# tky823/DNN-based_source_separation

Hardware: NVIDIA H100
Metric: audio-sec/s Conv-TasNet 2spk 4s@8kHz fwd+SI-SDR-PIT (higher is better)
Workload: dtype f32 via 3xFP16 split on wgmma (f16), fp32 accumulate

## Files before the change

### dnn-based_source_separation_b200/csrc/ctn_wgmma.cu

```cuda
#include "ctn_internal.h"
#include "ctn_wgmma_ptx.cuh"
#include "ctn_dw_math.cuh"
#include <cuda_fp16.h>
#include <stdlib.h>
#include <string.h>

int ctn_pw_simt(const PwArgs& a, int pro, int epi, cudaStream_t st);

namespace {

constexpr int TM = 128;
constexpr int KS = 32;
constexpr int NT = 128;
constexpr int THREADS = 256;
constexpr int CPW = 4;
constexpr int STAGES = 2;
constexpr int SMEM_HEADER = 1024;
constexpr int F16_MAX_ROWS = 2048;

template <int PRO, int EPI, bool F16>
__host__ __device__ constexpr bool chan_split() { return F16 && (PRO == PRO_DW || EPI == EPI_H); }
template <int PRO, int EPI, bool F16>
__host__ __device__ constexpr int tile_frames() { return chan_split<PRO, EPI, F16>() ? 64 : TM; }

struct TcArgs {
  PwArgs a;
  const float* wimg;
  const float* oscale;
  int n_tiles, k_slabs, t_tiles;
  int n_groups;
  int nt_per_cta;
};

template <int PRO>
__host__ __device__ constexpr int raw_q() { return PRO == PRO_DW ? 3 : PRO == PRO_RES ? 2 : 1; }
template <int PRO, int CPT>
struct Raw { float4 q[CPT][raw_q<PRO>()]; };

template <int PRO, int CPT>
__device__ __forceinline__ void load_raw(const PwArgs& a, int b, int c0, int tbase, int first, int step, bool interior, Raw<PRO, CPT>& r) {
#pragma unroll
  for (int j = 0; j < CPT; ++j) {
    const int c = c0 + j;
    if constexpr (PRO == PRO_DW) {
      const int cc = interior ? c : (c < a.K ? c : a.K - 1);
      const float* hr = a.A + ((size_t)b * a.K + cc) * a.pitch;
#pragma unroll
      for (int k = 0; k < 3; ++k) {
        int ts = first + k * step;
        if (!interior) ts = ts < 0 ? 0 : (ts > a.pitch - 4 ? a.pitch - 4 : ts);
        r.q[j][k] = __ldg(reinterpret_cast<const float4*>(hr + ts));
      }
    } else {
      const bool ok = c < a.K;
      r.q[j][0] = ok ? __ldg(reinterpret_cast<const float4*>(a.A + ((size_t)b * a.K + c) * a.pitch + tbase)) : make_float4(0.f, 0.f, 0.f, 0.f);
      if constexpr (PRO == PRO_RES)
        r.q[j][1] = ok ? __ldg(reinterpret_cast<const float4*>(a.res_r + ((size_t)b * a.res_Mt + c) * a.pitch + tbase))
                       : make_float4(0.f, 0.f, 0.f, 0.f);
    }
  }
}

template <int DCLS, bool INTERIOR, bool TRAIN, int CPT>
__device__ __forceinline__ void dw_form(const PwArgs& a, int b, int c0, int tbase, int first, int step, float2 mr1, float pslope,
                                        bool store_side, Raw<PRO_DW, CPT>& r, float4 (&v)[CPT], float2& dls, float2& dlss) {
  const float islope = TRAIN ? __ldg(a.dw_in_slope) : 0.f;
#pragma unroll
  for (int j = 0; j < CPT; ++j) {
    const int c = c0 + j;
    const int cc = INTERIOR ? c : (c < a.K ? c : a.K - 1);
    float4* q = r.q[j];
    if (TRAIN) {
#pragma unroll
      for (int k = 0; k < 3; ++k) {
        q[k].x = prelu_f(q[k].x, islope); q[k].y = prelu_f(q[k].y, islope); q[k].z = prelu_f(q[k].z, islope); q[k].w = prelu_f(q[k].w, islope);
      }
    }
    const float pg = __ldg(a.dw_norm_g + cc), pb = __ldg(a.dw_norm_b + cc), pbd = __ldg(a.dw_b + cc);
    const float w0 = __ldg(a.dw_w + cc * 3), w1 = __ldg(a.dw_w + cc * 3 + 1), w2 = __ldg(a.dw_w + cc * 3 + 2);
    const float gsc = pg * mr1.y, gsh = pb - mr1.x * mr1.y * pg;
    float4 pre;
    v[j] = dw_channel<DCLS, INTERIOR, TRAIN>(q[0], q[1], q[2], gsc, gsh, w0, w1, w2, pbd, pslope, first, step, tbase, a.frames, c < a.K,
                                             dls, dlss, &pre);
    if (TRAIN && store_side && c < a.K) *reinterpret_cast<float4*>(a.dw_u_pre_out + ((size_t)b * a.K + c) * a.pitch + tbase) = pre;
  }
}

template <int PRO, int EPI, int NPASS, bool F16, bool TRAIN>
__global__ void __launch_bounds__(THREADS, F16 ? 2 : 1) k_pw_wgmma(const TcArgs g) {
  constexpr bool CSPLIT = chan_split<PRO, EPI, F16>();
  constexpr int TMC = tile_frames<PRO, EPI, F16>();
  constexpr int NWG = CSPLIT ? 2 : 1;
  constexpr int LPR = TMC / 4;
  constexpr int CPT = CPW * LPR / 32;
  constexpr int NPREC = NPASS == 3 ? 2 : 1;
  constexpr uint32_t ROWB = F16 ? 64u : 128u;
  constexpr uint32_t A_BYTES = TMC * ROWB, W_BYTES = NT * ROWB;
  constexpr uint32_t STAGE_BYTES = NPREC * (A_BYTES + NWG * W_BYTES);
  static_assert(F16 || CPT == CPW, "the K-major tf32 store takes a warp's 4 channels per time step");
  extern __shared__ uint8_t smem_raw[];
  const uint32_t raw = ptx::smem_u32(smem_raw);
  const uint32_t base = (raw + 1023u) & ~1023u;
  uint8_t* smem = smem_raw + (base - raw);
  uint64_t* wbar = reinterpret_cast<uint64_t*>(smem);
  const uint32_t stage0 = base + SMEM_HEADER;
  const int warp = threadIdx.x >> 5, lane = threadIdx.x & 31, wg = warp >> 2;
  const PwArgs& a = g.a;

  const int n_groups = g.n_groups;
  const int ngrp = (int)blockIdx.x % n_groups;
  const int tt = ((int)blockIdx.x / n_groups) % g.t_tiles;
  const int b = (int)blockIdx.x / (n_groups * g.t_tiles);

  if (threadIdx.x == 0) {
    for (int s = 0; s < STAGES; ++s) ptx::mbar_init(ptx::smem_u32(&wbar[s]), 1);
    ptx::fence_mbar_init();
  }
  __syncthreads();

  float act_s = 1.f;
  if (F16 && a.act_scale) act_s = __ldg(a.act_scale);
  float pslope = 0.f;
  if (PRO == PRO_PRELU || PRO == PRO_DW) pslope = __ldg(a.pro_slope);
  const int c_thr = warp * CPW + (lane / LPR) * CPT;
  const int tbase = tt * TMC + (lane % LPR) * 4;
  float2 mr1 = make_float2(0.f, 1.f), mr_res = make_float2(0.f, 1.f);
  if (PRO == PRO_DW) mr1 = gln_mean_rstd(a.dw_stats_in + 2 * b, (double)a.K * (double)a.frames, a.dw_eps);
  if (PRO == PRO_RES) mr_res = gln_mean_rstd(a.res_stats + 2 * b, a.res_n, a.res_eps);
  int dcls = 4, first = tbase, step = 0;
  bool dw_interior = false;
  if (PRO == PRO_DW) {
    const int d = a.dw_dilation;
    dcls = d >= 4 ? 4 : d;
    step = dcls == 4 ? d : 4;
    first = dcls == 4 ? tbase - a.dw_pad_left : tbase - 4;
    const int reach = d >= 4 ? d : 4;
    dw_interior = (tt * TMC - reach >= 0) && (tt * TMC + TMC - 1 + reach + 3 < a.frames) && (a.K % KS == 0) && (a.dw_pad_left == d);
  }

  for (int ntl = 0; ntl < g.nt_per_cta; ++ntl) {
  const int nt0 = CSPLIT ? 2 * ngrp : ngrp * g.nt_per_cta + ntl;
  const int nt = CSPLIT ? nt0 + wg : nt0;
  const bool wg_live = nt < g.n_tiles;
  const int nw = CSPLIT ? min(2, g.n_tiles - nt0) : 1;
  const bool store_side = nt0 == 0;
  const uint8_t* wsrc = reinterpret_cast<const uint8_t*>(g.wimg) + (size_t)nt0 * g.k_slabs * NPREC * W_BYTES;
  float2 dls = make_float2(0.f, 0.f), dlss = make_float2(0.f, 0.f);
  float acc[64];
#pragma unroll
  for (int i = 0; i < 64; ++i) acc[i] = 0.f;

  Raw<PRO, CPT> cur;
  load_raw<PRO, CPT>(a, b, c_thr, tbase, first, step, dw_interior, cur);
  for (int ks = 0; ks < g.k_slabs; ++ks) {
    const int gk = ntl * g.k_slabs + ks;
    const int s = gk & 1;
    const uint32_t st_base = stage0 + (uint32_t)s * STAGE_BYTES;
    if (threadIdx.x == 0) {
      const uint32_t fb = ptx::smem_u32(&wbar[s]);
      ptx::mbar_arrive_expect_tx(fb, (uint32_t)nw * NPREC * W_BYTES);
      for (int w = 0; w < nw; ++w)
        ptx::bulk_g2s(st_base + NPREC * (A_BYTES + w * W_BYTES), wsrc + ((size_t)w * g.k_slabs + ks) * NPREC * W_BYTES, NPREC * W_BYTES, fb);
    }
    const int c0 = ks * KS + c_thr;
    float4 v[CPT];
    if constexpr (PRO == PRO_DW) {
      if (dw_interior) {
        if (dcls == 4) dw_form<4, true, TRAIN>(a, b, c0, tbase, first, step, mr1, pslope, store_side, cur, v, dls, dlss);
        else if (dcls == 2) dw_form<2, true, TRAIN>(a, b, c0, tbase, first, step, mr1, pslope, store_side, cur, v, dls, dlss);
        else dw_form<1, true, TRAIN>(a, b, c0, tbase, first, step, mr1, pslope, store_side, cur, v, dls, dlss);
      } else {
        if (dcls == 4) dw_form<4, false, TRAIN>(a, b, c0, tbase, first, step, mr1, pslope, store_side, cur, v, dls, dlss);
        else if (dcls == 2) dw_form<2, false, TRAIN>(a, b, c0, tbase, first, step, mr1, pslope, store_side, cur, v, dls, dlss);
        else dw_form<1, false, TRAIN>(a, b, c0, tbase, first, step, mr1, pslope, store_side, cur, v, dls, dlss);
      }
    } else {
#pragma unroll
      for (int j = 0; j < CPT; ++j) v[j] = cur.q[j][0];
      if (PRO == PRO_RES) {
#pragma unroll
        for (int j = 0; j < CPT; ++j) {
          const int k = c0 + j;
          const int kc = k < a.K ? k : a.K - 1;
          const float4 r = cur.q[j][PRO == PRO_RES ? 1 : 0];
          const float cst = __ldg(a.res_v1 + kc) - mr_res.x * mr_res.y * __ldg(a.res_v2 + kc);
          float4 xn;
          xn.x = fmaf(mr_res.y, r.x, v[j].x + cst); xn.y = fmaf(mr_res.y, r.y, v[j].y + cst);
          xn.z = fmaf(mr_res.y, r.z, v[j].z + cst); xn.w = fmaf(mr_res.y, r.w, v[j].w + cst);
          if (tbase + 0 >= a.frames) xn.x = 0.f;
          if (tbase + 1 >= a.frames) xn.y = 0.f;
          if (tbase + 2 >= a.frames) xn.z = 0.f;
          if (tbase + 3 >= a.frames) xn.w = 0.f;
          if (k >= a.K) xn = make_float4(0.f, 0.f, 0.f, 0.f);
          v[j] = xn;
          if (store_side && k < a.K) *reinterpret_cast<float4*>(a.res_x_out + ((size_t)b * a.K + k) * a.pitch + tbase) = xn;
        }
      }
      if (PRO == PRO_PRELU) {
#pragma unroll
        for (int j = 0; j < CPT; ++j) {
          v[j].x = prelu_f(v[j].x, pslope); v[j].y = prelu_f(v[j].y, pslope);
          v[j].z = prelu_f(v[j].z, pslope); v[j].w = prelu_f(v[j].w, pslope);
        }
      }
    }
    if (ks + 1 < g.k_slabs) load_raw<PRO, CPT>(a, b, (ks + 1) * KS + c_thr, tbase, first, step, dw_interior, cur);
    uint8_t* sa = smem + SMEM_HEADER + (size_t)s * STAGE_BYTES;
    if (F16) {
      const uint32_t f = (uint32_t)(tbase - tt * TMC);
#pragma unroll
      for (int j = 0; j < CPT; ++j) {
        const uint32_t c = (uint32_t)(c_thr + j);
        const uint32_t off = (f >> 6) * 4096u + (c >> 3) * 1024u + (c & 7) * 128u + ((((f >> 3) & 7) ^ (c & 7)) << 4) + (f & 7) * 2u;
        uint2 h2, l2;
        ptx::split_f16x2(v[j].x * act_s, v[j].y * act_s, h2.x, l2.x);
        ptx::split_f16x2(v[j].z * act_s, v[j].w * act_s, h2.y, l2.y);
        *reinterpret_cast<uint2*>(sa + off) = h2;
        *reinterpret_cast<uint2*>(sa + A_BYTES + off) = l2;
      }
    } else {
#pragma unroll
      for (int e = 0; e < 4; ++e) {
        const int t = lane * 4 + e;
        float x[CPW];
#pragma unroll
        for (int j = 0; j < CPW; ++j) x[j] = e == 0 ? v[j].x : e == 1 ? v[j].y : e == 2 ? v[j].z : v[j].w;
        const uint32_t off = (uint32_t)t * 128u + (((uint32_t)warp ^ (uint32_t)(t & 7)) << 4);
        float4 hi, lo;
        hi.x = ptx::hi_tf32(x[0]); hi.y = ptx::hi_tf32(x[1]); hi.z = ptx::hi_tf32(x[2]); hi.w = ptx::hi_tf32(x[3]);
        lo.x = x[0] - hi.x; lo.y = x[1] - hi.y; lo.z = x[2] - hi.z; lo.w = x[3] - hi.w;
        *reinterpret_cast<float4*>(sa + off) = hi;
        if (NPASS == 3) *reinterpret_cast<float4*>(sa + A_BYTES + off) = lo;
      }
    }
    ptx::fence_proxy_async_smem();
    __syncthreads();
    ptx::mbar_wait(ptx::smem_u32(&wbar[s]), (uint32_t)(gk >> 1) & 1u);
    if (wg_live) {
      const uint32_t a_hi = st_base + (CSPLIT ? 0u : (uint32_t)wg * 64u * ROWB), a_lo = a_hi + A_BYTES;
      const uint32_t w_hi = st_base + NPREC * (A_BYTES + (CSPLIT ? (uint32_t)wg * W_BYTES : 0u)), w_lo = w_hi + W_BYTES;
      ptx::wg_fence();
#pragma unroll
      for (int kk = 0; kk < (F16 ? KS / 16 : KS / 8); ++kk) {
        if (F16) {
          const uint64_t dah = ptx::wg_desc_mn128(a_hi + kk * 2048, 4096u, 1024u), dwh = ptx::wg_desc(w_hi + kk * 32, 8 * ROWB, ptx::SW64);
          ptx::wg_mma_f16(acc, dah, dwh);
          if (NPASS == 3) {
            const uint64_t dal = ptx::wg_desc_mn128(a_lo + kk * 2048, 4096u, 1024u), dwl = ptx::wg_desc(w_lo + kk * 32, 8 * ROWB, ptx::SW64);
            ptx::wg_mma_f16(acc, dal, dwh);
            ptx::wg_mma_f16(acc, dah, dwl);
          }
        } else {
          const uint64_t dah = ptx::wg_desc(a_hi + kk * 32, 8 * ROWB, ptx::SW128), dwh = ptx::wg_desc(w_hi + kk * 32, 8 * ROWB, ptx::SW128);
          ptx::wg_mma_tf32(acc, dah, dwh);
          if (NPASS == 3) {
            const uint64_t dal = ptx::wg_desc(a_lo + kk * 32, 8 * ROWB, ptx::SW128), dwl = ptx::wg_desc(w_lo + kk * 32, 8 * ROWB, ptx::SW128);
            ptx::wg_mma_tf32(acc, dal, dwh);
            ptx::wg_mma_tf32(acc, dah, dwl);
          }
        }
      }
      ptx::wg_commit();
      ptx::wg_wait<1>();
    }
    __syncthreads();
  }
  ptx::wg_wait<0>();

  if (PRO == PRO_DW && store_side) {
    const double sd = warp_sum_d((double)dls.x + (double)dls.y), ssd = warp_sum_d((double)dlss.x + (double)dlss.y);
    if (lane == 0) { atomicAdd(&a.dw_stats_out[2 * b], sd); atomicAdd(&a.dw_stats_out[2 * b + 1], ssd); }
  }
  if (!wg_live) continue;
  int n0 = nt * NT;
  asm volatile("" : "+r"(n0));

  float eslope = 0.f;
  if (EPI == EPI_H) eslope = __ldg(a.slope);
  const bool store_pre = EPI == EPI_H && a.store_pre != 0;
  float2 mr = make_float2(0.f, 1.f);
  if (EPI == EPI_HEAD) mr = gln_mean_rstd(a.stats_in + 2 * b, a.n_in, a.eps);
  const float inv_act = 1.f / act_s;
  const int row0 = (CSPLIT ? 0 : wg * 64) + (warp & 3) * 16 + (lane >> 2);
  float ls = 0.f, lss = 0.f;
#pragma unroll
  for (int i = 0; i < 64; ++i) {
    const int row = row0 + 8 * ((i >> 1) & 1);
    const int n = n0 + 8 * (i >> 2) + 2 * (lane & 3) + (i & 1);
    const int t = tt * TMC + row;
    if (n >= a.M) continue;
    const bool tvalid = t < a.frames;
    const float osc = F16 ? __ldg(g.oscale + n) * inv_act : 1.f;
    float v = acc[i];
    float* q = a.D + ((size_t)b * a.M + n) * a.pitch + t;
    if (EPI == EPI_RAW) {
      if (F16) v *= osc;
// ... 8 lines not shown
    } else if (EPI == EPI_MASK) {
      const float logit = F16 ? fmaf(v, osc, __ldg(a.bias + n)) : v + __ldg(a.bias + n);
      float mk;
      if (a.mask_logits) {
        mk = logit;
        v = logit;
      } else {
        mk = __fdividef(1.f, 1.f + __expf(-logit));
        v = tvalid ? mk * __ldg(a.wenc + ((size_t)b * a.Nb + n % a.Nb) * a.pitch + t) : 0.f;
      }
      if (a.mask_out) a.mask_out[((size_t)b * a.M + n) * a.pitch + t] = tvalid ? mk : 0.f;
    }
    *q = tvalid ? v : 0.f;
  }
  if (EPI == EPI_H) {
    const double s = warp_sum_d((double)ls), ss = warp_sum_d((double)lss);
    if (lane == 0) { atomicAdd(&a.stats_out[2 * b], s); atomicAdd(&a.stats_out[2 * b + 1], ss); }
  }
  }
}

constexpr int MD_MAX_K = 128;
constexpr int MD_STAGES = 4;
constexpr int MD_ROW = 20;
constexpr uint32_t MD_A_BYTES = TM * 64u, MD_W_BYTES = NT * 64u;
constexpr int MD_TAB = NT * 16 + 2 * NT;
constexpr size_t MD_SMEM = 1024 + SMEM_HEADER + (size_t)(MD_MAX_K / KS) * 2 * MD_A_BYTES + (size_t)MD_STAGES * 2 * MD_W_BYTES +
                           (size_t)TM * MD_ROW * sizeof(float) + 2 * (size_t)MD_TAB * sizeof(float);

__global__ void __launch_bounds__(THREADS, 1) k_maskdec(const TcArgs g) {
  extern __shared__ uint8_t smem_raw[];
  const uint32_t raw = ptx::smem_u32(smem_raw);
  const uint32_t base = (raw + 1023u) & ~1023u;
  uint8_t* smem = smem_raw + (base - raw);
  uint64_t* wbar = reinterpret_cast<uint64_t*>(smem);
  const uint32_t op0 = base + SMEM_HEADER;
  const uint32_t ring0 = op0 + (uint32_t)(MD_MAX_K / KS) * 2 * MD_A_BYTES;
  float* dacc = reinterpret_cast<float*>(smem + (ring0 - base) + MD_STAGES * 2 * MD_W_BYTES);
  float* tab0 = dacc + TM * MD_ROW;
  const int warp = threadIdx.x >> 5, lane = threadIdx.x & 31, wg = warp >> 2;
  const PwArgs& a = g.a;
  const int tt = (int)blockIdx.x % g.t_tiles, b = (int)blockIdx.x / g.t_tiles;
  const int ntps = a.Nb / NT, n_tiles = g.n_tiles, k_slabs = g.k_slabs;
  const int total = n_tiles * k_slabs;
  const uint8_t* wimg = reinterpret_cast<const uint8_t*>(g.wimg);

  for (int i = threadIdx.x; i < TM * MD_ROW; i += THREADS) dacc[i] = 0.f;
  if (threadIdx.x == 0) {
    for (int s = 0; s < MD_STAGES; ++s) ptx::mbar_init(ptx::smem_u32(&wbar[s]), 1);
    ptx::fence_mbar_init();
  }
  __syncthreads();
  int issued = 0;
  auto refill = [&](int consumed) {
    for (; issued < total && issued < consumed + MD_STAGES; ++issued) {
      const uint32_t fb = ptx::smem_u32(&wbar[issued % MD_STAGES]);
      ptx::mbar_arrive_expect_tx(fb, 2 * MD_W_BYTES);
      ptx::bulk_g2s(ring0 + (uint32_t)(issued % MD_STAGES) * 2 * MD_W_BYTES, wimg + (size_t)issued * 2 * MD_W_BYTES, 2 * MD_W_BYTES, fb);
    }
  };
  if (threadIdx.x == 0) refill(0);

  const float act_s = __ldg(a.act_scale), pslope = __ldg(a.pro_slope);
  {
    const int tbase = tt * TM + lane * 4;
    float4 v[MD_MAX_K / KS][CPW];
#pragma unroll
    for (int ks = 0; ks < MD_MAX_K / KS; ++ks)
#pragma unroll
      for (int j = 0; j < CPW; ++j) {
        const int c = ks * KS + warp * CPW + j;
        v[ks][j] = ks < k_slabs && c < a.K ? __ldg(reinterpret_cast<const float4*>(a.A + ((size_t)b * a.K + c) * a.pitch + tbase))
                                           : make_float4(0.f, 0.f, 0.f, 0.f);
      }
    const uint32_t f = (uint32_t)lane * 4u;
#pragma unroll
    for (int ks = 0; ks < MD_MAX_K / KS; ++ks) {
      if (ks >= k_slabs) break;
      uint8_t* sa = smem + (op0 - base) + (size_t)ks * 2 * MD_A_BYTES;
#pragma unroll
      for (int j = 0; j < CPW; ++j) {
        float4 x = v[ks][j];
        x.x = prelu_f(x.x, pslope); x.y = prelu_f(x.y, pslope); x.z = prelu_f(x.z, pslope); x.w = prelu_f(x.w, pslope);
        const uint32_t c = (uint32_t)(warp * CPW + j);
        const uint32_t off = (f >> 6) * 4096u + (c >> 3) * 1024u + (c & 7) * 128u + ((((f >> 3) & 7) ^ (c & 7)) << 4) + (f & 7) * 2u;
        uint2 h2, l2;
        ptx::split_f16x2(x.x * act_s, x.y * act_s, h2.x, l2.x);
        ptx::split_f16x2(x.z * act_s, x.w * act_s, h2.y, l2.y);
        *reinterpret_cast<uint2*>(sa + off) = h2;
        *reinterpret_cast<uint2*>(sa + MD_A_BYTES + off) = l2;
      }
    }
  }
  ptx::fence_proxy_async_smem();
  __syncthreads();

  const float inv_act = 1.f / act_s;
  const int row0 = wg * 64 + (warp & 3) * 16 + (lane >> 2);
  const int t0 = tt * TM + row0;
  const int S = a.M / a.Nb;
  for (int nt = 0; nt < n_tiles; ++nt) {
    const int src = nt / ntps, nb0 = (nt - src * ntps) * NT;
    float wv[64];
    {
      const float* wr = a.wenc + ((size_t)b * a.Nb + nb0 + 2 * (lane & 3)) * a.pitch + t0;
#pragma unroll
      for (int i = 0; i < 64; ++i) wv[i] = __ldg(wr + (size_t)(8 * (i >> 2) + (i & 1)) * a.pitch + 8 * ((i >> 1) & 1));
    }
    const int tc = threadIdx.x & (NT - 1), th = threadIdx.x >> 7;
    const float4* dsrc = reinterpret_cast<const float4*>(a.dec_w + (size_t)(nb0 + tc) * 16) + 2 * th;
    const float4 td0 = __ldg(dsrc), td1 = __ldg(dsrc + 1);
    const float tsb = th == 0 ? __ldg(g.oscale + nt * NT + tc) * inv_act : __ldg(a.bias + nt * NT + tc);
    float acc[64];
#pragma unroll
    for (int i = 0; i < 64; ++i) acc[i] = 0.f;
    for (int ks = 0; ks < k_slabs; ++ks) {
      const int q = nt * k_slabs + ks;
      const uint32_t w_hi = ring0 + (uint32_t)(q % MD_STAGES) * 2 * MD_W_BYTES, w_lo = w_hi + MD_W_BYTES;
      const uint32_t a_hi = op0 + (uint32_t)ks * 2 * MD_A_BYTES + (uint32_t)wg * 4096u, a_lo = a_hi + MD_A_BYTES;
      ptx::mbar_wait(ptx::smem_u32(&wbar[q % MD_STAGES]), (uint32_t)(q / MD_STAGES) & 1u);
      ptx::wg_fence();
#pragma unroll
      for (int kk = 0; kk < KS / 16; ++kk) {
        const uint64_t dah = ptx::wg_desc_mn128(a_hi + kk * 2048, 4096u, 1024u), dwh = ptx::wg_desc(w_hi + kk * 32, 8 * 64, ptx::SW64);
        const uint64_t dal = ptx::wg_desc_mn128(a_lo + kk * 2048, 4096u, 1024u), dwl = ptx::wg_desc(w_lo + kk * 32, 8 * 64, ptx::SW64);
        ptx::wg_mma_f16(acc, dah, dwh);
        ptx::wg_mma_f16(acc, dal, dwh);
        ptx::wg_mma_f16(acc, dah, dwl);
      }
      ptx::wg_commit();
    }
    ptx::wg_wait<0>();
    float* tab = tab0 + (nt & 1) * MD_TAB;
    float4* tdec = reinterpret_cast<float4*>(tab);
    tdec[(2 * th) * NT + tc] = td0;
    tdec[(2 * th + 1) * NT + tc] = td1;
    tab[NT * 16 + th * NT + tc] = tsb;
    __syncthreads();
    if (threadIdx.x == 0) refill((nt + 1) * k_slabs);

    float dpart[2][16];
#pragma unroll
    for (int k = 0; k < 32; ++k) dpart[k >> 4][k & 15] = 0.f;
#pragma unroll
    for (int i = 0; i < 64; ++i) {
      const int c = 8 * (i >> 2) + 2 * (lane & 3) + (i & 1);
      const bool tvalid = t0 + 8 * ((i >> 1) & 1) < a.frames;
      const float osc = tab[NT * 16 + c];
      const float logit = fmaf(acc[i], osc, tab[NT * 17 + c]);
      const float o = tvalid ? __fdividef(wv[i], 1.f + __expf(-logit)) : 0.f;
#pragma unroll
      for (int q4 = 0; q4 < 4; ++q4) {
        const float4 d4 = tdec[q4 * NT + c];
        float* dp = dpart[(i >> 1) & 1] + 4 * q4;
        dp[0] = fmaf(o, d4.x, dp[0]); dp[1] = fmaf(o, d4.y, dp[1]); dp[2] = fmaf(o, d4.z, dp[2]); dp[3] = fmaf(o, d4.w, dp[3]);
      }
    }
    const bool hb0 = lane & 1, hb1 = lane & 2;
    float r1[16];
#pragma unroll
    for (int j = 0; j < 16; ++j) {
      const float keep = hb0 ? dpart[1][j] : dpart[0][j], send = hb0 ? dpart[0][j] : dpart[1][j];
      r1[j] = keep + __shfl_xor_sync(0xffffffffu, send, 1);
    }
    float r2[8];
#pragma unroll
    for (int j = 0; j < 8; ++j) {
      const float keep = hb1 ? r1[8 + j] : r1[j], send = hb1 ? r1[j] : r1[8 + j];
      r2[j] = keep + __shfl_xor_sync(0xffffffffu, send, 2);
    }
    float4* dst = reinterpret_cast<float4*>(dacc + (row0 + (hb0 ? 8 : 0)) * MD_ROW + (hb1 ? 8 : 0));
    float4 u0 = dst[0], u1 = dst[1];
    u0.x += r2[0]; u0.y += r2[1]; u0.z += r2[2]; u0.w += r2[3];
    u1.x += r2[4]; u1.y += r2[5]; u1.z += r2[6]; u1.w += r2[7];
    dst[0] = u0; dst[1] = u1;

    if (nt - src * ntps == ntps - 1) {
      __syncthreads();
      float* yo = a.D + ((size_t)b * S + src) * (size_t)a.dec_T_out;
      const long long tb = 8LL * tt * TM - a.dec_crop_left;
      for (int j = threadIdx.x; j < 2 * 32 * (TM / 8 + 1); j += THREADS) {
        const int u = j >> 5, f = (u >> 1) * 8 + 2 * ((j & 31) >> 3) + (u & 1), k = j & 7;
        if (f > TM) continue;
        const int sidx = 8 * f + k;
        float v = 0.f;
        if (f < TM) { v += dacc[f * MD_ROW + k]; dacc[f * MD_ROW + k] = 0.f; }
        if (f >= 1) { v += dacc[(f - 1) * MD_ROW + 8 + k]; dacc[(f - 1) * MD_ROW + 8 + k] = 0.f; }
        const long long tau = tb + sidx;
        if (tau < 0 || tau >= a.dec_T_out) continue;
        if (sidx < 8 || sidx >= 8 * TM) atomicAdd(yo + tau, v);
        else yo[tau] = v;
      }
    }
  }
}

__host__ __device__ __forceinline__ int wimg_offset(int nl, int kl) {
  return (nl >> 3) * 256 + (nl & 7) * 32 + ((((kl >> 2) ^ (nl & 7)) << 2) | (kl & 3));
}

__device__ __forceinline__ void wimg_f16_group(const float* __restrict__ W, int M, int K, int n_tile, int k_slabs, int nt, int grp,
                                               __half* __restrict__ img, float* __restrict__ oscale, float* smax) {
  static_assert(KS == 32, "one lane per channel of a slab");
  const int lane = threadIdx.x & 31, wid = threadIdx.x >> 5;
  const int nl = grp * 16 + wid;
  const int n = nt * n_tile + nl;
  const bool live = nl < n_tile && n < M;
  const float* row = W + (size_t)n * K;
  float mx = 0.f;
  if (live)
    for (int k = lane; k < K; k += 32) mx = fmaxf(mx, fabsf(row[k]));
#pragma unroll
  for (int o = 16; o > 0; o >>= 1) mx = fmaxf(mx, __shfl_xor_sync(0xffffffffu, mx, o));
  if (lane == 0) smax[wid] = mx;
  __syncthreads();
  mx = smax[lane & 15];
#pragma unroll
  for (int o = 8; o > 0; o >>= 1) mx = fmaxf(mx, __shfl_xor_sync(0xffffffffu, mx, o));
  __syncthreads();
  int e = 0;
  if (mx > 0.f && mx < INFINITY) e = 9 - ilogbf(mx);
  e = max(-100, min(100, e));
  const float up = ldexpf(1.f, e), down = ldexpf(1.f, -e);
  if (nl >= n_tile) return;
  if (lane == 0) oscale[n] = down;
  const size_t per = (size_t)n_tile * KS;
  for (int ks = 0; ks < k_slabs; ++ks) {
    const int kl = lane, k = ks * KS + kl;
    const float x = (live && k < K) ? row[k] * up : 0.f;
    __half* dst = img + ((size_t)nt * k_slabs + ks) * 2 * per;
    const int off = (nl >> 3) * 256 + (nl & 7) * 32 + ((((kl >> 3) ^ ((nl >> 1) & 3))) << 3) + (kl & 7);
    const __half hi = __float2half_rn(x);
    dst[off] = hi;
    dst[per + off] = __float2half_rn(x - __half2float(hi));
  }
}
__host__ __device__ inline size_t wimg_f16_image_bytes(int n_tile, int n_tiles, int k_slabs) {
  return (size_t)n_tiles * k_slabs * 2 * n_tile * KS * sizeof(__half);
}

struct WimgJobs { WimgJob j[CTN_MAX_JOBS]; };
__device__ __forceinline__ void wimg_tf32_slab(const float* __restrict__ W, int M, int K, int k_slabs, int nt, int ks, int nprec,
                                               float* __restrict__ wimg) {
  const int n_tile = NT;
  const size_t per = (size_t)n_tile * KS;
  float* dst = wimg + ((size_t)nt * k_slabs + ks) * nprec * per;
  for (int i = threadIdx.x; i < n_tile * KS; i += 256) {
    const int nl = i / KS, kl = i % KS;
    const int n = nt * n_tile + nl, k = ks * KS + kl;
    const float x = (n < M && k < K) ? W[(size_t)n * K + k] : 0.f;
    const int off = wimg_offset(nl, kl);
    const float hi = ptx::to_tf32(x);
    dst[off] = hi;
    if (nprec == 2) dst[per + off] = ptx::to_tf32(x - hi);
  }
}

__global__ void __launch_bounds__(256) k_build_wimg_batch(const WimgJobs jobs, int nprec) {
  const WimgJob& jb = jobs.j[blockIdx.y];
  const int n_tiles = (jb.M + NT - 1) / NT, k_slabs = (jb.K + KS - 1) / KS;
  const int blk = blockIdx.x;
  if (blk >= n_tiles * k_slabs) return;
  const int nt = blk / k_slabs, ks = blk - nt * k_slabs;
  wimg_tf32_slab(jb.W, jb.M, jb.K, k_slabs, nt, ks, nprec, jb.wimg);
}

__global__ void __launch_bounds__(512) k_build_wimg_batch_f16(const WimgJobs jobs) {
  __shared__ float smax[16];
  const WimgJob& jb = jobs.j[blockIdx.y];
  const int n_tile = NT;
  const int n_tiles = (jb.M + n_tile - 1) / n_tile, k_slabs = (jb.K + KS - 1) / KS;
  const int groups = n_tile / 16;
  __half* img = reinterpret_cast<__half*>(jb.wimg);
  float* oscale = reinterpret_cast<float*>(reinterpret_cast<uint8_t*>(jb.wimg) + wimg_f16_image_bytes(n_tile, n_tiles, k_slabs));
  for (int blk = blockIdx.x; blk < n_tiles * groups; blk += gridDim.x)
    wimg_f16_group(jb.W, jb.M, jb.K, n_tile, k_slabs, blk / groups, blk % groups, img, oscale, smax);
}

int eff_math(int M, int math) {
  if (math != CTN_MATH_F16X3) return math;
  return ((M + NT - 1) / NT) * NT > F16_MAX_ROWS ? CTN_MATH_TF32X3 : math;
}

template <int PRO, int EPI, int NPASS, bool F16, bool TRAIN>
int launch(const TcArgs& g0, cudaStream_t st) {
  constexpr int NPREC = NPASS == 3 ? 2 : 1;
  constexpr bool CSPLIT = chan_split<PRO, EPI, F16>();
  constexpr int TMC = tile_frames<PRO, EPI, F16>();
  constexpr size_t smem = SMEM_HEADER + 1024 + (size_t)STAGES * NPREC * (TMC + (CSPLIT ? 2 : 1) * NT) * (F16 ? 64 : 128);
  TcArgs g = g0;
  g.t_tiles = g.a.pitch / TMC;
  g.n_groups = CSPLIT ? (g.n_tiles + 1) / 2 : g.n_tiles / g.nt_per_cta;
  static bool attr_done[CTN_MAX_DEVICES] = {false};
  const int dev = ctn_current_device();
  if (!attr_done[dev]) {
    cudaError_t e = cudaFuncSetAttribute(k_pw_wgmma<PRO, EPI, NPASS, F16, TRAIN>, cudaFuncAttributeMaxDynamicSharedMemorySize, (int)smem);
    if (e != cudaSuccess) return (int)e;
    attr_done[dev] = true;
  }
  const long long grid = (long long)g.a.B * g.t_tiles * g.n_groups;
  if (grid > 0x7fffffffLL) return CTN_EUNSUPPORTED;
  k_pw_wgmma<PRO, EPI, NPASS, F16, TRAIN><<<(unsigned)grid, THREADS, smem, st>>>(g);
  CTN_COUNT_LAUNCH();
  CTN_RETURN_IF_CUDA_ERR();
  return CTN_OK;
}

template <int PRO, int EPI, bool TRAIN = false>
int launch_math(const TcArgs& g, int math, cudaStream_t st) {
  if (math == CTN_MATH_F16X3) return launch<PRO, EPI, 3, true, TRAIN>(g, st);
  if (math == CTN_MATH_TF32) return launch<PRO, EPI, 1, false, TRAIN>(g, st);
  return launch<PRO, EPI, 3, false, TRAIN>(g, st);
}

int piece_math(int math, bool bounded) { return math == CTN_MATH_F16X3 && !bounded ? CTN_MATH_TF32X3 : math; }

int build_images(const WimgJob* jobs, int n, int math, cudaStream_t st) {
  const bool f16 = math == CTN_MATH_F16X3;
  for (int i0 = 0; i0 < n; i0 += CTN_MAX_JOBS) {
    WimgJobs wj;
    const int m = n - i0 < CTN_MAX_JOBS ? n - i0 : CTN_MAX_JOBS;
    int maxb = 1;
    for (int i = 0; i < m; ++i) {
      const WimgJob& jb = jobs[i0 + i];
      wj.j[i] = jb;
      const int blocks = ((jb.M + NT - 1) / NT) * (f16 ? NT / 16 : (jb.K + KS - 1) / KS);
      if (blocks > maxb) maxb = blocks;
    }
    if (f16) k_build_wimg_batch_f16<<<dim3(maxb, m), 512, 0, st>>>(wj);
    else k_build_wimg_batch<<<dim3(maxb, m), 256, 0, st>>>(wj, math == CTN_MATH_TF32 ? 1 : 2);
    CTN_COUNT_LAUNCH();
  }
  CTN_RETURN_IF_CUDA_ERR();
  return CTN_OK;
}

bool maskdec_ok(const PwArgs& a, int pmath) {
  return eff_math(a.M, pmath) == CTN_MATH_F16X3 && a.dec_w && a.Nb > 0 && a.Nb % NT == 0 && a.M % a.Nb == 0 && a.K <= MD_MAX_K &&
         (((uintptr_t)a.dec_w) & 15) == 0;
}

int launch_maskdec(const TcArgs& g0, cudaStream_t st) {
  TcArgs g = g0;
  g.t_tiles = g.a.pitch / TM;
  g.n_groups = 1;
  static bool attr_done[CTN_MAX_DEVICES] = {false};
  const int dev = ctn_current_device();
  if (!attr_done[dev]) {
    cudaError_t e = cudaFuncSetAttribute(k_maskdec, cudaFuncAttributeMaxDynamicSharedMemorySize, (int)MD_SMEM);
    if (e != cudaSuccess) return (int)e;
    attr_done[dev] = true;
  }
  const long long grid = (long long)g.a.B * g.t_tiles;
  if (grid > 0x7fffffffLL) return CTN_EUNSUPPORTED;
  k_maskdec<<<(unsigned)grid, THREADS, MD_SMEM, st>>>(g);
  CTN_COUNT_LAUNCH();
  CTN_RETURN_IF_CUDA_ERR();
  return CTN_OK;
}

int launch_wgmma(const PwArgs& a, int pro, int epi, int pmath, cudaStream_t st) {
  if (!a.wimg) return CTN_EINVAL;
  const int math = eff_math(a.M, pmath);
  if (a.pitch % TM != 0) return CTN_EALIGN;
  if ((((uintptr_t)a.A) | ((uintptr_t)a.wimg)) & 15) return CTN_EALIGN;
  TcArgs g;
  g.a = a;
  g.wimg = a.wimg;
  g.n_tiles = (a.M + NT - 1) / NT;
  g.k_slabs = (a.K + KS - 1) / KS;
  g.oscale = math == CTN_MATH_F16X3
                 ? reinterpret_cast<const float*>(reinterpret_cast<const uint8_t*>(a.wimg) + wimg_f16_image_bytes(NT, g.n_tiles, g.k_slabs))
                 : nullptr;
  g.nt_per_cta = 1;
  const bool train_dw = pro == PRO_DW && a.dw_u_pre_out != nullptr;
  if (pro == PRO_NONE && epi == EPI_RAW) return launch_math<PRO_NONE, EPI_RAW>(g, math, st);
  if (pro == PRO_DW && epi == EPI_RAW)
    return train_dw ? launch_math<PRO_DW, EPI_RAW, true>(g, math, st) : launch_math<PRO_DW, EPI_RAW>(g, math, st);
  if (pro == PRO_NONE && epi == EPI_HEAD) return launch_math<PRO_NONE, EPI_HEAD>(g, math, st);
  if (pro == PRO_NONE && epi == EPI_H) return launch_math<PRO_NONE, EPI_H>(g, math, st);
  if (pro == PRO_RES && epi == EPI_H) return launch_math<PRO_RES, EPI_H>(g, math, st);
  if (pro == PRO_PRELU && epi == EPI_MASK) return launch_math<PRO_PRELU, EPI_MASK>(g, math, st);
  if (pro == PRO_PRELU && epi == EPI_MASKDEC) {
    if (!maskdec_ok(a, pmath)) return CTN_EUNSUPPORTED;
    return launch_maskdec(g, st);
  }
  return CTN_EUNSUPPORTED;
}

}

extern "C" int ctn_has_tcgen05(void) { return 1; }

size_t ctn_pw_wimg_bytes(int M, int K, int math) {
  const int nprec = math == CTN_MATH_TF32 ? 1 : 2;
  const int n_tiles = (M + NT - 1) / NT, k_slabs = (K + KS - 1) / KS;
  return (size_t)n_tiles * k_slabs * nprec * NT * KS * sizeof(float) + (size_t)n_tiles * NT * sizeof(float) + 256;
}

size_t ctn_pw_wimg_max_bytes(const int (*shapes)[2], int n, int math) {
  if (math == CTN_MATH_FP32) return 256;
  size_t mx = 0;
  for (int i = 0; i < n; ++i) {
    const size_t b = ctn_pw_wimg_bytes(shapes[i][0], shapes[i][1], math);
    if (b > mx) mx = b;
  }
  return mx;
}

int ctn_pw_prepare(const PwArgs& a, int math, float* wimg, cudaStream_t st) {
  const WimgJob job{a.W, wimg, a.M, a.K};
  return ctn_pw_prepare_batch(&job, 1, math, a.act_scale != nullptr, st);
}

int ctn_pw_prepare_batch(const WimgJob* jobs, int n, int math, bool bounded, cudaStream_t st) {
  if (math == CTN_MATH_FP32) return CTN_OK;
  math = piece_math(math, bounded);
  bool uniform = true;
  for (int i = 0; i < n; ++i) uniform = uniform && eff_math(jobs[i].M, math) == math;
  if (uniform) return build_images(jobs, n, math, st);
  for (int i = 0; i < n; ++i) CTN_TRY(build_images(jobs + i, 1, eff_math(jobs[i].M, math), st));
  return CTN_OK;
}

int ctn_pw_maskdec_supported(const PwArgs& a, int math) { return maskdec_ok(a, piece_math(math, a.act_scale != nullptr)); }

int ctn_pw(const PwArgs& a, int pro, int epi, int math, float* wimg_scratch, cudaStream_t st) {
  if (math == CTN_MATH_FP32) return ctn_pw_simt(a, pro, epi, st);
  const int pmath = piece_math(math, a.act_scale != nullptr);
  if (!wimg_scratch) return launch_wgmma(a, pro, epi, pmath, st);
  CTN_TRY(ctn_pw_prepare(a, math, wimg_scratch, st));
  PwArgs b = a;
  b.wimg = wimg_scratch;
  return launch_wgmma(b, pro, epi, pmath, st);
}
```

### dnn-based_source_separation_b200/csrc/ctn_wgmma_ptx.cuh

```cuda
#pragma once
#include <cuda_runtime.h>
#include <stdint.h>

namespace ptx {

__device__ __forceinline__ uint32_t smem_u32(const void* p) { return (uint32_t)__cvta_generic_to_shared(p); }

__device__ __forceinline__ void mbar_init(uint32_t bar, uint32_t count) {
  asm volatile("mbarrier.init.shared::cta.b64 [%0], %1;" ::"r"(bar), "r"(count) : "memory");
}
__device__ __forceinline__ void fence_mbar_init() { asm volatile("fence.mbarrier_init.release.cluster;" ::: "memory"); }
__device__ __forceinline__ void mbar_arrive(uint32_t bar) {
  asm volatile("mbarrier.arrive.shared::cta.b64 _, [%0];" ::"r"(bar) : "memory");
}
__device__ __forceinline__ void mbar_arrive_expect_tx(uint32_t bar, uint32_t bytes) {
  asm volatile("mbarrier.arrive.expect_tx.shared::cta.b64 _, [%0], %1;" ::"r"(bar), "r"(bytes) : "memory");
}
__device__ __forceinline__ void mbar_wait(uint32_t bar, uint32_t parity) {
  asm volatile(
      "{\n\t"
      ".reg .pred P1;\n\t"
      "LAB_WAIT:\n\t"
      "mbarrier.try_wait.parity.shared::cta.b64 P1, [%0], %1;\n\t"
      "@P1 bra DONE;\n\t"
      "bra LAB_WAIT;\n\t"
      "DONE:\n\t"
      "}" ::"r"(bar), "r"(parity) : "memory");
}

__device__ __forceinline__ void fence_proxy_async_smem() { asm volatile("fence.proxy.async.shared::cta;" ::: "memory"); }

__device__ __forceinline__ void bulk_g2s(uint32_t dst_smem, const void* src, uint32_t bytes, uint32_t bar) {
  asm volatile("cp.async.bulk.shared::cluster.global.mbarrier::complete_tx::bytes [%0], [%1], %2, [%3];" ::"r"(dst_smem),
               "l"(src), "r"(bytes), "r"(bar)
               : "memory");
}

__device__ __forceinline__ void bulk_g2s_multicast(uint32_t dst_smem, const void* src, uint32_t bytes, uint32_t bar, uint16_t cta_mask) {
  asm volatile(
      "cp.async.bulk.shared::cluster.global.mbarrier::complete_tx::bytes.multicast::cluster [%0], [%1], %2, [%3], %4;" ::"r"(dst_smem),
      "l"(src), "r"(bytes), "r"(bar), "h"(cta_mask)
      : "memory");
}

__device__ __forceinline__ bool elect_one() {
  uint32_t pred = 0;
  asm volatile(
      "{\n\t"
      ".reg .b32 rx;\n\t"
      ".reg .pred px;\n\t"
      "elect.sync rx|px, 0xFFFFFFFF;\n\t"
      "@px mov.s32 %0, 1;\n\t"
      "}"
      : "+r"(pred));
  return pred != 0;
}

__device__ __forceinline__ uint32_t cluster_ctarank() {
  uint32_t r;
  asm volatile("mov.u32 %0, %%cluster_ctarank;" : "=r"(r));
  return r;
}
__device__ __forceinline__ void cluster_sync_all() {
  asm volatile("barrier.cluster.arrive.release.aligned;" ::: "memory");
  asm volatile("barrier.cluster.wait.acquire.aligned;" ::: "memory");
}

__device__ __forceinline__ void mbar_arrive_remote(uint32_t local_bar, uint32_t rank) {
  asm volatile(
      "{\n\t"
      ".reg .b32 ra;\n\t"
      "mapa.shared::cluster.u32 ra, %0, %1;\n\t"
      "mbarrier.arrive.release.cluster.shared::cluster.b64 _, [ra];\n\t"
      "}" ::"r"(local_bar), "r"(rank)
      : "memory");
}
__device__ __forceinline__ void mbar_wait_cluster(uint32_t bar, uint32_t parity) {
  asm volatile(
      "{\n\t"
      ".reg .pred P1;\n\t"
      "LAB_WAIT:\n\t"
      "mbarrier.try_wait.parity.acquire.cluster.shared::cta.b64 P1, [%0], %1;\n\t"
      "@P1 bra DONE;\n\t"
      "bra LAB_WAIT;\n\t"
      "DONE:\n\t"
      "}" ::"r"(bar), "r"(parity) : "memory");
}

__device__ __forceinline__ void bulk_s2peer(uint32_t dst_smem, uint32_t src_smem, uint32_t bytes, uint32_t bar, uint32_t rank) {
  asm volatile(
      "{\n\t"
      ".reg .b32 rd, rb;\n\t"
      "mapa.shared::cluster.u32 rd, %0, %4;\n\t"
      "mapa.shared::cluster.u32 rb, %3, %4;\n\t"
      "cp.async.bulk.shared::cluster.shared::cta.mbarrier::complete_tx::bytes [rd], [%1], %2, [rb];\n\t"
      "}" ::"r"(dst_smem), "r"(src_smem), "r"(bytes), "r"(bar), "r"(rank)
      : "memory");
}

__device__ __forceinline__ void st_peer_v4(uint32_t local_addr, uint32_t rank, uint32_t a, uint32_t b, uint32_t c, uint32_t d) {
  asm volatile(
      "{\n\t"
      ".reg .b32 ra;\n\t"
      "mapa.shared::cluster.u32 ra, %0, %1;\n\t"
      "st.shared::cluster.v4.b32 [ra], {%2, %3, %4, %5};\n\t"
      "}" ::"r"(local_addr), "r"(rank), "r"(a), "r"(b), "r"(c), "r"(d)
      : "memory");
}

__device__ __forceinline__ void wg_fence() { asm volatile("wgmma.fence.sync.aligned;" ::: "memory"); }
// ... 51 lines not shown
```

Before: 7857.

## Add activation-resident pointwise-1 wgmma kernel streaming weights across N tiles

Adds a specialised kernel for the first pointwise conv (EPI_H, f16x3, K<=128). Each CTA loads its whole 64-frame activation tile once into shared memory as split f16 hi/lo operands. The two warpgroups then loop over alternating output-channel tiles, streaming weights through a per-warpgroup bulk-copy ring synchronised by named barriers. This replaces the generic per-N-tile kernel, which reloaded and resplit the activations for every tile, at the cost of more shared memory per CTA and a larger CTA that covers all N tiles. The residual prologue and the swizzle offset are factored into shared helpers.

```diff
diff --git a/dnn-based_source_separation_b200/csrc/ctn_wgmma.cu b/dnn-based_source_separation_b200/csrc/ctn_wgmma.cu
--- a/dnn-based_source_separation_b200/csrc/ctn_wgmma.cu
+++ b/dnn-based_source_separation_b200/csrc/ctn_wgmma.cu
@@ -59,6 +59,32 @@
                        : make_float4(0.f, 0.f, 0.f, 0.f);
     }
   }
+}
+
+template <int CPT>
+__device__ __forceinline__ void res_form(const PwArgs& a, int b, int c0, int tbase, float2 mr_res, bool store, const Raw<PRO_RES, CPT>& cur,
+                                         float4 (&v)[CPT]) {
+#pragma unroll
+  for (int j = 0; j < CPT; ++j) {
+    const int k = c0 + j;
+    const int kc = k < a.K ? k : a.K - 1;
+    const float4 x = cur.q[j][0], r = cur.q[j][1];
+    const float cst = __ldg(a.res_v1 + kc) - mr_res.x * mr_res.y * __ldg(a.res_v2 + kc);
+    float4 xn;
+    xn.x = fmaf(mr_res.y, r.x, x.x + cst); xn.y = fmaf(mr_res.y, r.y, x.y + cst);
+    xn.z = fmaf(mr_res.y, r.z, x.z + cst); xn.w = fmaf(mr_res.y, r.w, x.w + cst);
+    if (tbase + 0 >= a.frames) xn.x = 0.f;
+    if (tbase + 1 >= a.frames) xn.y = 0.f;
+    if (tbase + 2 >= a.frames) xn.z = 0.f;
+    if (tbase + 3 >= a.frames) xn.w = 0.f;
+    if (k >= a.K) xn = make_float4(0.f, 0.f, 0.f, 0.f);
+    v[j] = xn;
+    if (store && k < a.K) *reinterpret_cast<float4*>(a.res_x_out + ((size_t)b * a.K + k) * a.pitch + tbase) = xn;
+  }
+}
+
+__device__ __forceinline__ uint32_t mn128_offset(uint32_t f, uint32_t c) {
+  return (f >> 6) * 4096u + (c >> 3) * 1024u + (c & 7) * 128u + ((((f >> 3) & 7) ^ (c & 7)) << 4) + (f & 7) * 2u;
 }
 
 template <int DCLS, bool INTERIOR, bool TRAIN, int CPT>
@@ -177,25 +203,7 @@
     } else {
 #pragma unroll
       for (int j = 0; j < CPT; ++j) v[j] = cur.q[j][0];
-      if (PRO == PRO_RES) {
-#pragma unroll
-        for (int j = 0; j < CPT; ++j) {
-          const int k = c0 + j;
-          const int kc = k < a.K ? k : a.K - 1;
-          const float4 r = cur.q[j][PRO == PRO_RES ? 1 : 0];
-          const float cst = __ldg(a.res_v1 + kc) - mr_res.x * mr_res.y * __ldg(a.res_v2 + kc);
-          float4 xn;
-          xn.x = fmaf(mr_res.y, r.x, v[j].x + cst); xn.y = fmaf(mr_res.y, r.y, v[j].y + cst);
-          xn.z = fmaf(mr_res.y, r.z, v[j].z + cst); xn.w = fmaf(mr_res.y, r.w, v[j].w + cst);
-          if (tbase + 0 >= a.frames) xn.x = 0.f;
-          if (tbase + 1 >= a.frames) xn.y = 0.f;
-          if (tbase + 2 >= a.frames) xn.z = 0.f;
-          if (tbase + 3 >= a.frames) xn.w = 0.f;
-          if (k >= a.K) xn = make_float4(0.f, 0.f, 0.f, 0.f);
-          v[j] = xn;
-          if (store_side && k < a.K) *reinterpret_cast<float4*>(a.res_x_out + ((size_t)b * a.K + k) * a.pitch + tbase) = xn;
-        }
-      }
+      if constexpr (PRO == PRO_RES) res_form<CPT>(a, b, c0, tbase, mr_res, store_side, cur, v);
       if (PRO == PRO_PRELU) {
 #pragma unroll
         for (int j = 0; j < CPT; ++j) {
@@ -210,8 +218,7 @@
       const uint32_t f = (uint32_t)(tbase - tt * TMC);
 #pragma unroll
       for (int j = 0; j < CPT; ++j) {
-        const uint32_t c = (uint32_t)(c_thr + j);
-        const uint32_t off = (f >> 6) * 4096u + (c >> 3) * 1024u + (c & 7) * 128u + ((((f >> 3) & 7) ^ (c & 7)) << 4) + (f & 7) * 2u;
+        const uint32_t off = mn128_offset(f, (uint32_t)(c_thr + j));
         uint2 h2, l2;
         ptx::split_f16x2(v[j].x * act_s, v[j].y * act_s, h2.x, l2.x);
         ptx::split_f16x2(v[j].z * act_s, v[j].w * act_s, h2.y, l2.y);
@@ -386,8 +393,7 @@
       for (int j = 0; j < CPW; ++j) {
         float4 x = v[ks][j];
         x.x = prelu_f(x.x, pslope); x.y = prelu_f(x.y, pslope); x.z = prelu_f(x.z, pslope); x.w = prelu_f(x.w, pslope);
-        const uint32_t c = (uint32_t)(warp * CPW + j);
-        const uint32_t off = (f >> 6) * 4096u + (c >> 3) * 1024u + (c & 7) * 128u + ((((f >> 3) & 7) ^ (c & 7)) << 4) + (f & 7) * 2u;
+        const uint32_t off = mn128_offset(f, (uint32_t)(warp * CPW + j));
         uint2 h2, l2;
         ptx::split_f16x2(x.x * act_s, x.y * act_s, h2.x, l2.x);
         ptx::split_f16x2(x.z * act_s, x.w * act_s, h2.y, l2.y);
@@ -496,6 +502,163 @@
         else yo[tau] = v;
       }
     }
+  }
+}
+
+constexpr int P1_MAX_K = 128;
+constexpr int P1_TF = 64;
+constexpr int P1_WST = 2;
+constexpr uint32_t P1_A_BYTES = P1_TF * 64u, P1_W_BYTES = NT * 64u;
+constexpr size_t P1_SMEM = 1024 + SMEM_HEADER + (size_t)(P1_MAX_K / KS) * 2 * P1_A_BYTES + (size_t)2 * P1_WST * 2 * P1_W_BYTES +
+                           (size_t)2 * 2 * 2 * NT * sizeof(float) + (size_t)(THREADS / 32) * 2 * sizeof(double);
+
+__device__ __forceinline__ void wg_bar(int wg) {
+  if (wg == 0) ptx::named_bar_sync<1, 128>();
+  else ptx::named_bar_sync<2, 128>();
+}
+
+template <int PRO>
+__global__ void __launch_bounds__(THREADS, 2) k_pw1_resident(const TcArgs g) {
+  static_assert(PRO == PRO_NONE || PRO == PRO_RES, "pw1 prologues");
+  constexpr int NSL = P1_MAX_K / KS;
+  constexpr int CPT = 2;
+  extern __shared__ uint8_t smem_raw[];
+  const uint32_t raw = ptx::smem_u32(smem_raw);
+  const uint32_t base = (raw + 1023u) & ~1023u;
+  uint8_t* smem = smem_raw + (base - raw);
+  uint64_t* wbar = reinterpret_cast<uint64_t*>(smem);
+  const uint32_t op0 = base + SMEM_HEADER;
+  const uint32_t ring0 = op0 + (uint32_t)NSL * 2 * P1_A_BYTES;
+  float* tab0 = reinterpret_cast<float*>(smem + (ring0 - base) + 2 * P1_WST * 2 * P1_W_BYTES);
+  double* red = reinterpret_cast<double*>(tab0 + 2 * 2 * 2 * NT);
+  const int warp = threadIdx.x >> 5, lane = threadIdx.x & 31, wg = warp >> 2, lt = threadIdx.x & (NT - 1);
+  const PwArgs& a = g.a;
+  const int tt = (int)blockIdx.x % g.t_tiles, b = (int)blockIdx.x / g.t_tiles;
+  const int k_slabs = g.k_slabs;
+  const int passes = g.n_tiles > wg ? (g.n_tiles - wg + 1) / 2 : 0;
+  const int total = passes * k_slabs;
+  const uint8_t* wimg = reinterpret_cast<const uint8_t*>(g.wimg);
+  const uint32_t ring = ring0 + (uint32_t)wg * P1_WST * 2 * P1_W_BYTES;
+
+  if (threadIdx.x == 0) {
+    for (int s = 0; s < 2 * P1_WST; ++s) ptx::mbar_init(ptx::smem_u32(&wbar[s]), 1);
+    ptx::fence_mbar_init();
+  }
+  __syncthreads();
+  int issued = 0;
+  auto refill = [&](int consumed) {
+    for (; issued < total && issued < consumed + P1_WST; ++issued) {
+      const int p = issued / k_slabs, ks = issued - p * k_slabs;
+      const uint32_t fb = ptx::smem_u32(&wbar[wg * P1_WST + issued % P1_WST]);
+      ptx::mbar_arrive_expect_tx(fb, 2 * P1_W_BYTES);
+      ptx::bulk_g2s(ring + (uint32_t)(issued % P1_WST) * 2 * P1_W_BYTES, wimg + ((size_t)(2 * p + wg) * k_slabs + ks) * 2 * P1_W_BYTES,
+                    2 * P1_W_BYTES, fb);
+    }
+  };
+  if (lt == 0) refill(0);
+
+  const float act_s = __ldg(a.act_scale);
+  {
+    const int c_thr = warp * CPW + (lane / 16) * CPT;
+    const int tbase = tt * P1_TF + (lane % 16) * 4;
+    Raw<PRO, CPT> cur[NSL];
+#pragma unroll
+    for (int ks = 0; ks < NSL; ++ks)
+      if (ks < k_slabs) load_raw<PRO, CPT>(a, b, ks * KS + c_thr, tbase, 0, 0, false, cur[ks]);
+    float2 mr_res = make_float2(0.f, 1.f);
+    if (PRO == PRO_RES) mr_res = gln_mean_rstd(a.res_stats + 2 * b, a.res_n, a.res_eps);
+    const uint32_t f = (uint32_t)(tbase - tt * P1_TF);
+#pragma unroll
+    for (int ks = 0; ks < NSL; ++ks) {
+      if (ks >= k_slabs) break;
+      float4 v[CPT];
+      if constexpr (PRO == PRO_RES) {
+        res_form<CPT>(a, b, ks * KS + c_thr, tbase, mr_res, true, cur[ks], v);
+      } else {
+#pragma unroll
+        for (int j = 0; j < CPT; ++j) v[j] = cur[ks].q[j][0];
+      }
+      uint8_t* sa = smem + (op0 - base) + (size_t)ks * 2 * P1_A_BYTES;
+#pragma unroll
+      for (int j = 0; j < CPT; ++j) {
+        const uint32_t off = mn128_offset(f, (uint32_t)(c_thr + j));
+        uint2 h2, l2;
+        ptx::split_f16x2(v[j].x * act_s, v[j].y * act_s, h2.x, l2.x);
+        ptx::split_f16x2(v[j].z * act_s, v[j].w * act_s, h2.y, l2.y);
+        *reinterpret_cast<uint2*>(sa + off) = h2;
+        *reinterpret_cast<uint2*>(sa + P1_A_BYTES + off) = l2;
+      }
+    }
+  }
+  ptx::fence_proxy_async_smem();
+  __syncthreads();
+
+  const float inv_act = 1.f / act_s, eslope = __ldg(a.slope);
+  const bool store_pre = a.store_pre != 0;
+  const int row0 = (warp & 3) * 16 + (lane >> 2);
+  double cs = 0.0, css = 0.0;
+  for (int p = 0; p < passes; ++p) {
+    const int nt = 2 * p + wg;
+    const int tn = nt * NT + lt;
+    const float tsc = tn < a.M ? __ldg(g.oscale + tn) * inv_act : 0.f;
+    const float tbi = tn < a.M ? __ldg(a.bias + tn) : 0.f;
+    float acc[64];
+#pragma unroll
+    for (int i = 0; i < 64; ++i) acc[i] = 0.f;
+    for (int ks = 0; ks < k_slabs; ++ks) {
+      const int u = p * k_slabs + ks;
+      const uint32_t w_hi = ring + (uint32_t)(u % P1_WST) * 2 * P1_W_BYTES, w_lo = w_hi + P1_W_BYTES;
+      const uint32_t a_hi = op0 + (uint32_t)ks * 2 * P1_A_BYTES, a_lo = a_hi + P1_A_BYTES;
+      ptx::mbar_wait(ptx::smem_u32(&wbar[wg * P1_WST + u % P1_WST]), (uint32_t)(u / P1_WST) & 1u);
+      ptx::wg_fence();
+#pragma unroll
+      for (int kk = 0; kk < KS / 16; ++kk) {
+        const uint64_t dah = ptx::wg_desc_mn128(a_hi + kk * 2048, 4096u, 1024u), dwh = ptx::wg_desc(w_hi + kk * 32, 8 * 64, ptx::SW64);
+        const uint64_t dal = ptx::wg_desc_mn128(a_lo + kk * 2048, 4096u, 1024u), dwl = ptx::wg_desc(w_lo + kk * 32, 8 * 64, ptx::SW64);
+        ptx::wg_mma_f16(acc, dah, dwh);
+        ptx::wg_mma_f16(acc, dal, dwh);
+        ptx::wg_mma_f16(acc, dah, dwl);
+      }
+      ptx::wg_commit();
+      if (ks > 0) {
+        ptx::wg_wait<1>();
+        wg_bar(wg);
+        if (lt == 0) refill(u);
+      }
+    }
+    ptx::wg_wait<0>();
+    float* tab = tab0 + (wg * 2 + (p & 1)) * 2 * NT;
+    tab[lt] = tsc;
+    tab[NT + lt] = tbi;
+    wg_bar(wg);
+    if (lt == 0) refill((p + 1) * k_slabs);
+
+    int n0 = nt * NT;
+    asm volatile("" : "+r"(n0));
+    float ls = 0.f, lss = 0.f;
+#pragma unroll
+    for (int i = 0; i < 64; ++i) {
+      const int row = row0 + 8 * ((i >> 1) & 1);
+      const int c = 8 * (i >> 2) + 2 * (lane & 3) + (i & 1);
+      const int n = n0 + c;
+      const int t = tt * P1_TF + row;
+      if (n >= a.M) continue;
+      const bool tvalid = t < a.frames;
+      const float pre = fmaf(acc[i], tab[c], tab[NT + c]);
+      const float act = prelu_f(pre, eslope);
+      if (tvalid) { ls += act; lss = fmaf(act, act, lss); }
+      a.D[((size_t)b * a.M + n) * a.pitch + t] = tvalid ? (store_pre ? pre : act) : 0.f;
+    }
+    cs += warp_sum_d((double)ls);
+    css += warp_sum_d((double)lss);
+  }
+  if (lane == 0) { red[2 * warp] = cs; red[2 * warp + 1] = css; }
+  __syncthreads();
+  if (threadIdx.x == 0) {
+    double s = 0.0, ss = 0.0;
+    for (int w = 0; w < THREADS / 32; ++w) { s += red[2 * w]; ss += red[2 * w + 1]; }
+    atomicAdd(&a.stats_out[2 * b], s);
+    atomicAdd(&a.stats_out[2 * b + 1], ss);
   }
 }
 
@@ -658,6 +821,26 @@
   const long long grid = (long long)g.a.B * g.t_tiles;
   if (grid > 0x7fffffffLL) return CTN_EUNSUPPORTED;
   k_maskdec<<<(unsigned)grid, THREADS, MD_SMEM, st>>>(g);
+  CTN_COUNT_LAUNCH();
+  CTN_RETURN_IF_CUDA_ERR();
+  return CTN_OK;
+}
+
+template <int PRO>
+int launch_pw1(const TcArgs& g0, cudaStream_t st) {
+  TcArgs g = g0;
+  g.t_tiles = g.a.pitch / P1_TF;
+  g.n_groups = 1;
+  static bool attr_done[CTN_MAX_DEVICES] = {false};
+  const int dev = ctn_current_device();
+  if (!attr_done[dev]) {
+    cudaError_t e = cudaFuncSetAttribute(k_pw1_resident<PRO>, cudaFuncAttributeMaxDynamicSharedMemorySize, (int)P1_SMEM);
+    if (e != cudaSuccess) return (int)e;
+    attr_done[dev] = true;
+  }
+  const long long grid = (long long)g.a.B * g.t_tiles;
+  if (grid > 0x7fffffffLL) return CTN_EUNSUPPORTED;
+  k_pw1_resident<PRO><<<(unsigned)grid, THREADS, P1_SMEM, st>>>(g);
   CTN_COUNT_LAUNCH();
   CTN_RETURN_IF_CUDA_ERR();
   return CTN_OK;
@@ -682,6 +865,10 @@
   if (pro == PRO_DW && epi == EPI_RAW)
     return train_dw ? launch_math<PRO_DW, EPI_RAW, true>(g, math, st) : launch_math<PRO_DW, EPI_RAW>(g, math, st);
   if (pro == PRO_NONE && epi == EPI_HEAD) return launch_math<PRO_NONE, EPI_HEAD>(g, math, st);
+  if (epi == EPI_H && math == CTN_MATH_F16X3 && a.K <= P1_MAX_K) {
+    if (pro == PRO_NONE) return launch_pw1<PRO_NONE>(g, st);
+    if (pro == PRO_RES) return launch_pw1<PRO_RES>(g, st);
+  }
   if (pro == PRO_NONE && epi == EPI_H) return launch_math<PRO_NONE, EPI_H>(g, math, st);
   if (pro == PRO_RES && epi == EPI_H) return launch_math<PRO_RES, EPI_H>(g, math, st);
   if (pro == PRO_PRELU && epi == EPI_MASK) return launch_math<PRO_PRELU, EPI_MASK>(g, math, st);
diff --git a/dnn-based_source_separation_b200/csrc/ctn_wgmma_ptx.cuh b/dnn-based_source_separation_b200/csrc/ctn_wgmma_ptx.cuh
--- a/dnn-based_source_separation_b200/csrc/ctn_wgmma_ptx.cuh
+++ b/dnn-based_source_separation_b200/csrc/ctn_wgmma_ptx.cuh
@@ -26,6 +26,11 @@
       "bra LAB_WAIT;\n\t"
       "DONE:\n\t"
       "}" ::"r"(bar), "r"(parity) : "memory");
+}
+
+template <uint32_t ID, uint32_t THREADS>
+__device__ __forceinline__ void named_bar_sync() {
+  asm volatile("bar.sync %0, %1;" ::"n"(ID), "n"(THREADS) : "memory");
 }
 
 __device__ __forceinline__ void fence_proxy_async_smem() { asm volatile("fence.proxy.async.shared::cta;" ::: "memory"); }
```

Result: faster. 8460 (median of 6 runs) (+7.7%).
